# ylsung/vl-merging

Hardware: AMD Instinct MI355X
Metric: VL samples/sec (fwd+bwd) base_vl 384^2 at 1/2/4/8 GPUs; merge GB/s vs HBM peak (higher is better)
Workload: dtype bf16

## Files before the change

### include/vlm_hip.h

```cpp
#ifndef VLM_HIP_H
#define VLM_HIP_H
#include <stddef.h>
#include <stdint.h>

#ifdef __cplusplus
extern "C" {
#endif

#define VLM_OK 0
#define VLM_ERR_ARG (-1)
#define VLM_ERR_LAUNCH (-2)
#define VLM_ERR_WORKSPACE (-3)
#define VLM_ERR_UNSUPPORTED (-4)

#define VLM_ABI_VERSION 10
int vlm_abi_version(void);
int vlm_device_cus(void);
int vlm_set_cu_budget(int cus);
int vlm_debug_occupy(int workgroups, int threads, int lds_bytes, int microseconds, void* stream);

#define VLM_MERGE_LERP 0
#define VLM_MERGE_TASKVEC 1
#define VLM_MERGE_MEAN 2
#define VLM_MERGE_MAX_SRC 4
// ... 10 lines not shown

size_t vlm_merge_plan_bytes(int n_jobs, uint64_t total_elems);
int vlm_merge_plan_upload(const vlm_merge_job_t* jobs_host, int n_jobs, void* workspace, size_t workspace_bytes,
                          void* stream);
int vlm_merge_run(const void* workspace, void* stream);

#define VLM_ACT_NONE 0
#define VLM_ACT_GELU 1
#define VLM_ACT_GELU_BWD 2
#define VLM_ACT_GELU_DERIV 3
#define VLM_ACT_MUL_AUX 4

typedef struct {
  const float* bias;
  const float* col_scale;
  const float* row_scale;
  const float* residual;
  int64_t ld_res;
  void* aux;
  int64_t ld_aux;
  int32_t act;
  float alpha;
  int32_t accumulate;
  int32_t reserved;
  float* col_sum;
  float* col_sum_ws;
  float* splitk_ws;
  uint64_t splitk_ws_bytes;
} vlm_epilogue_t;

int vlm_gemm_bf16(int ta, int tb, int M, int N, int K, const void* A, int lda, const void* B, int ldb, void* C,
                  int ldc, int c_is_f32, const vlm_epilogue_t* epi, void* stream);
#define VLM_GEMM_MAX_GROUPS 4
typedef struct {
  int32_t row0, rows;
  const void* B;
  int32_t ldb;
  int32_t reserved;
  const float* bias;
  float* col_sum;
  float* col_sum_ws;
} vlm_gemm_group_t;
int vlm_gemm_bf16_grouped(int n_groups, const vlm_gemm_group_t* groups, int N, int K, const void* A, int lda, void* C,
                          int ldc, int c_is_f32, const vlm_epilogue_t* epi, void* stream);
typedef struct {
  int32_t row0, rows;
  float* C;
  int32_t accumulate;
  int32_t reserved;
} vlm_wgrad_group_t;
int vlm_gemm_wgrad_grouped(int n_groups, const vlm_wgrad_group_t* groups, int M, int N, const void* A, int lda,
                           const void* B, int ldb, int ldc, float* splitk_ws, uint64_t splitk_ws_bytes, void* stream);
int vlm_gemm_set_big_tile_mode(int mode);

int vlm_layernorm_fwd(const float* x, int ldx, int M, int D, const float* gamma, const float* beta, float eps,
                      void* y, int ldy, int y_is_f32, float* stats, void* stream);
#define VLM_ROW_WS_BYTES(D) ((size_t)1536 * 2 * (size_t)(D) * sizeof(float))
int vlm_layernorm_bwd(const void* dy, int lddy, int dy_is_f32, const float* x, int ldx, const float* stats,
                      const float* gamma, int M, int D, const float* dres, int lddres, float* dx, int lddx,
                      float* dgamma, float* dbeta, float* workspace, size_t workspace_bytes, int* deferred_blocks,
                      void* stream);
typedef struct {
  const void* y;
  int32_t ldy;
  const float* gamma;
  const float* row_scale;
  void* dy;
  int32_t lddy;
  float* dgamma;
  float* dbias;
  float* workspace;
  size_t workspace_bytes;
} vlm_layerscale_t;
int vlm_layernorm_bwd_scale(const void* dy, int lddy, int dy_is_f32, const float* x, int ldx, const float* stats,
                            const float* gamma, int M, int D, const float* dres, int lddres, float* dx, int lddx,
                            float* dgamma, float* dbeta, float* workspace, size_t workspace_bytes,
                            const vlm_layerscale_t* scale, int* deferred_blocks, void* stream);
#define VLM_MAX_FOLD_JOBS 16
typedef struct {
  const float* partials;
  int32_t nblocks;
  int32_t D;
  float* out0;
  float* out1;
} vlm_fold_job_t;
int vlm_colreduce_batch(const vlm_fold_job_t* jobs_host, int n_jobs, void* stream);
int vlm_layerscale_bwd(const float* dx, int lddx, const void* y_bf16, int ldy, const float* gamma,
                       const float* row_scale, int M, int D, void* dy_bf16, int lddy, float* dgamma, float* dbias,
                       float* workspace, size_t workspace_bytes, int* deferred_blocks, void* stream);
#define VLM_MAX_LAYERSCALE_JOBS 32
typedef struct {
  const float* weight;
  const float* gamma;
  const float* bias;
  void* shadow;
  float* bias_out;
  float* raw_w;
  float* raw_b;
  float* dweight;
  float* dbias;
  float* dgamma;
  int32_t N, K;
} vlm_layerscale_job_t;
int vlm_layerscale_fold(const vlm_layerscale_job_t* jobs_host, int n_jobs, void* stream);
int vlm_layerscale_finish(const vlm_layerscale_job_t* jobs_host, int n_jobs, void* stream);
int vlm_colsum_bf16(const void* a, int lda, int M, int N, float* out, void* stream);
// ... 125 lines not shown
```

### vl-merging_amd/_lib.py

```python
import ctypes
import os

_HERE = os.path.dirname(os.path.abspath(__file__))
LIB_PATH = os.environ.get("VLM_LIB_PATH") or os.path.join(_HERE, "lib", "libvlm_hip.so")
_lib = None

c_void_p = ctypes.c_void_p
c_int = ctypes.c_int
c_float = ctypes.c_float
c_size_t = ctypes.c_size_t
c_u64 = ctypes.c_uint64

MERGE_LERP, MERGE_TASKVEC, MERGE_MEAN = 0, 1, 2
MERGE_MAX_SRC = 4


class MergeJob(ctypes.Structure):
    _fields_ = [
        ("dst", c_void_p),
        ("base", c_void_p),
        ("src", c_void_p * MERGE_MAX_SRC),
        ("ratio", c_float * MERGE_MAX_SRC),
        ("n_src", ctypes.c_int32),
        ("mode", ctypes.c_int32),
# ... 57 lines not shown
        ("B", ctypes.c_int32), ("n0", ctypes.c_int32), ("n1", ctypes.c_int32), ("base0", ctypes.c_int32),
        ("base1", ctypes.c_int32), ("pos1", ctypes.c_int32), ("scale", c_float), ("reserved", ctypes.c_int32),
        ("bias_dense", c_void_p), ("bias_dense_t", c_void_p), ("dense_tiles", ctypes.c_int32), ("reserved2", ctypes.c_int32),
    ]


class LayerScaleJob(ctypes.Structure):
    _fields_ = [("weight", c_void_p), ("gamma", c_void_p), ("bias", c_void_p), ("shadow", c_void_p), ("bias_out", c_void_p),
                ("raw_w", c_void_p), ("raw_b", c_void_p), ("dweight", c_void_p), ("dbias", c_void_p), ("dgamma", c_void_p),
                ("N", ctypes.c_int32), ("K", ctypes.c_int32)]


MAX_LAYERSCALE_JOBS = 32


class VlmError(RuntimeError):
    pass


_ERR = {-1: "VLM_ERR_ARG", -2: "VLM_ERR_LAUNCH", -3: "VLM_ERR_WORKSPACE", -4: "VLM_ERR_UNSUPPORTED"}

SIGNATURES = {
    "vlm_abi_version": (c_int, []),
    "vlm_device_cus": (c_int, []),
    "vlm_set_cu_budget": (c_int, [c_int]),
    "vlm_debug_occupy": (c_int, [c_int, c_int, c_int, c_int, c_void_p]),
    "vlm_layerscale_fold": (c_int, [ctypes.POINTER(LayerScaleJob), c_int, c_void_p]),
    "vlm_layerscale_finish": (c_int, [ctypes.POINTER(LayerScaleJob), c_int, c_void_p]),
    "vlm_merge_plan_bytes": (c_size_t, [c_int, c_u64]),
    "vlm_merge_plan_upload": (c_int, [ctypes.POINTER(MergeJob), c_int, c_void_p, c_size_t, c_void_p]),
    "vlm_merge_run": (c_int, [c_void_p, c_void_p]),
    "vlm_gemm_bf16": (c_int, [c_int, c_int, c_int, c_int, c_int, c_void_p, c_int, c_void_p, c_int, c_void_p, c_int,
                              c_int, ctypes.POINTER(Epilogue), c_void_p]),
    "vlm_gemm_bf16_grouped": (c_int, [c_int, ctypes.POINTER(GemmGroup), c_int, c_int, c_void_p, c_int, c_void_p, c_int, c_int,
                                      ctypes.POINTER(Epilogue), c_void_p]),
    "vlm_gemm_wgrad_grouped": (c_int, [c_int, ctypes.POINTER(WgradGroup), c_int, c_int, c_void_p, c_int, c_void_p, c_int, c_int,
                                       c_void_p, c_u64, c_void_p]),
    "vlm_attention_fwd": (c_int, [ctypes.POINTER(AttnDesc), c_void_p, c_int, c_void_p, c_void_p]),
    "vlm_attention_bwd_ws_floats": (c_size_t, [ctypes.POINTER(AttnDesc), c_int]),
    "vlm_attention_bwd": (c_int, [ctypes.POINTER(AttnDesc), c_void_p, c_int, c_void_p, c_int, c_void_p, c_void_p, c_size_t,
                                  c_void_p, c_int, c_void_p, c_void_p, c_void_p]),
    "vlm_layernorm_fwd": (c_int, [c_void_p, c_int, c_int, c_int, c_void_p, c_void_p, c_float, c_void_p, c_int, c_int,
                                  c_void_p, c_void_p]),
    "vlm_layernorm_bwd": (c_int, [c_void_p, c_int, c_int, c_void_p, c_int, c_void_p, c_void_p, c_int, c_int, c_void_p,
                                  c_int, c_void_p, c_int, c_void_p, c_void_p, c_void_p, c_size_t,
                                  ctypes.POINTER(c_int), c_void_p]),
    "vlm_layernorm_bwd_scale": (c_int, [c_void_p, c_int, c_int, c_void_p, c_int, c_void_p, c_void_p, c_int, c_int, c_void_p,
                                        c_int, c_void_p, c_int, c_void_p, c_void_p, c_void_p, c_size_t,
                                        ctypes.POINTER(LayerScale), ctypes.POINTER(c_int), c_void_p]),
    "vlm_layerscale_bwd": (c_int, [c_void_p, c_int, c_void_p, c_int, c_void_p, c_void_p, c_int, c_int, c_void_p, c_int,
                                   c_void_p, c_void_p, c_void_p, c_size_t, ctypes.POINTER(c_int), c_void_p]),
    "vlm_colreduce_batch": (c_int, [ctypes.POINTER(FoldJob), c_int, c_void_p]),
    "vlm_gemm_set_big_tile_mode": (c_int, [c_int]),
    "vlm_colsum_bf16": (c_int, [c_void_p, c_int, c_int, c_int, c_void_p, c_void_p]),
    "vlm_adamw_step": (c_int, [c_void_p, c_void_p, c_void_p, c_void_p, c_void_p, c_u64, c_float, c_float, c_float,
                               c_float, c_float, c_float, c_float, c_int, c_void_p]),
    "vlm_accumulate_f32_f64": (c_int, [c_void_p, c_void_p, c_u64, c_void_p]),
    "vlm_gram_f64": (c_int, [c_void_p, c_int, c_int, c_int, c_int, c_void_p, c_void_p]),
    "vlm_gemm_f64": (c_int, [c_int, c_int, c_int, c_int, c_int, ctypes.c_double, c_void_p, c_int, c_int, c_void_p, c_int,
                             ctypes.c_double, c_void_p, c_int, c_void_p]),
    "vlm_scale_gram_f64": (c_int, [c_void_p, c_void_p, c_int, ctypes.c_double, c_int, c_void_p]),
    "vlm_potrf_block_f64": (c_int, [c_void_p, c_int, c_int, c_int, c_void_p, c_void_p]),
    "vlm_trsm_block_f64": (c_int, [c_void_p, c_int, c_int, c_int, c_int, c_void_p, c_int, c_int, c_int, c_void_p]),
    "vlm_cholesky_f64": (c_int, [c_void_p, c_int, c_void_p, c_void_p]),
    "vlm_solve_spd_right_f64": (c_int, [c_void_p, c_int, c_void_p, c_int, c_int, c_void_p]),
    "vlm_gemm_f64_batched": (c_int, [c_int, c_int, c_int, c_int, c_int, ctypes.c_double, ctypes.POINTER(c_void_p), c_int, c_int,
                                     ctypes.POINTER(c_void_p), c_int, ctypes.c_double, ctypes.POINTER(c_void_p), c_int, c_int, c_void_p]),
    "vlm_cholesky_f64_batched": (c_int, [ctypes.POINTER(c_void_p), c_int, c_int, c_void_p, c_void_p]),
    "vlm_solve_spd_right_f64_batched": (c_int, [ctypes.POINTER(c_void_p), c_int, ctypes.POINTER(c_void_p), c_int, c_int, c_int, c_void_p]),
    "vlm_cross_entropy_fwd": (c_int, [c_void_p, c_int, c_int, c_int, c_void_p, ctypes.c_int64, c_void_p, c_void_p, c_void_p]),
    "vlm_cross_entropy_bwd": (c_int, [c_void_p, c_int, c_int, c_int, c_void_p, ctypes.c_int64, c_void_p, c_void_p, c_void_p, c_int,
                                      c_void_p]),
    "vlm_l2norm_fwd": (c_int, [c_void_p, c_int, c_int, c_int, c_int, c_void_p, c_void_p, c_void_p]),
    "vlm_l2norm_bwd": (c_int, [c_void_p, c_void_p, c_void_p, c_int, c_int, c_void_p, c_int, c_int, c_void_p]),
    "vlm_contrastive_ws_floats": (c_size_t, [c_int]),
    "vlm_contrastive": (c_int, [c_void_p, c_void_p, c_int, c_int, c_int, c_void_p, c_void_p, c_void_p, c_void_p, c_void_p, c_void_p,
                                c_void_p]),
    "vlm_small_cross_entropy": (c_int, [c_void_p, c_int, c_int, c_int, c_int, c_void_p, c_void_p, c_void_p, c_void_p]),
    "vlm_cross_entropy_reduce": (c_int, [c_void_p, c_void_p, c_int, c_int, ctypes.c_int64, c_void_p, c_void_p]),
    "vlm_scale_by_scalar": (c_int, [ctypes.POINTER(c_void_p), ctypes.POINTER(c_void_p), ctypes.POINTER(c_int), c_int, c_void_p, c_void_p]),
    "vlm_text_rows_fwd": (c_int, [c_void_p, c_int, c_void_p, c_int, c_void_p, c_void_p, c_void_p, c_float, c_void_p, c_float, c_float,
                                  c_void_p, c_void_p, c_int, c_void_p, c_int, c_void_p]),
    "vlm_text_rows_bwd_ws_floats": (c_size_t, [c_int]),
    "vlm_text_rows_bwd": (c_int, [c_void_p, c_int, c_void_p, c_int, c_void_p, c_int, c_void_p, c_void_p, c_void_p, c_void_p, c_float, c_float,
                                  c_int, c_void_p, ctypes.c_int64, c_void_p, c_void_p, c_void_p, c_void_p, c_void_p, c_void_p]),
    "vlm_image_rows_prep": (c_int, [c_void_p, c_void_p, c_void_p, c_int, c_void_p, c_void_p]),
    "vlm_image_lead_rows": (c_int, [c_void_p, c_int, c_int, c_int, c_int, c_void_p, c_void_p]),
    "vlm_image_rows_bwd_ws_floats": (c_size_t, [c_int]),
    "vlm_image_rows_bwd": (c_int, [c_void_p, c_int, c_int, c_int, c_int, c_void_p, c_void_p, c_void_p, c_void_p, c_void_p, c_void_p]),
    "vlm_tanh_fwd": (c_int, [c_void_p, c_int, c_int, c_int, c_void_p, c_void_p]),
    "vlm_act_bwd": (c_int, [c_void_p, c_int, c_int, c_void_p, c_int, c_int, c_int, c_int, c_int, c_void_p, c_void_p]),
    "vlm_colsum_small": (c_int, [c_void_p, c_int, c_int, c_int, c_void_p, c_void_p]),
    "vlm_sample_negatives": (c_int, [c_void_p, c_int, c_int, c_void_p, c_int, c_int, c_int, c_int, c_void_p, c_void_p, c_void_p]),
    "vlm_weighted_sum": (c_int, [ctypes.POINTER(c_void_p), ctypes.POINTER(c_float), c_int, c_void_p, c_void_p]),
    "vlm_scatter_rows": (c_int, [c_void_p, c_int, c_int, c_int, c_int, c_void_p, c_int, c_void_p]),
    "vlm_cast_f32_bf16": (c_int, [c_void_p, c_void_p, c_u64, c_void_p]),
    "vlm_embedding_bwd": (c_int, [c_void_p, c_int, c_void_p, ctypes.c_int64, c_int, ctypes.c_int64, c_void_p, c_int,
                                  ctypes.c_int64, c_void_p]),
    "vlm_bias_dense_bytes": (c_size_t, [c_int, c_int, c_int, c_int]),
    "vlm_bias_dense": (c_int, [c_void_p, c_int, c_int, c_void_p, c_int, c_int, c_int, c_int, c_int, c_int, c_void_p,
                               c_void_p]),
    "vlm_transpose_bf16_tiles": (c_int, [c_void_p, c_int, c_void_p]),
    "vlm_droppath_sites": (c_int, [c_void_p, c_void_p, c_void_p, c_int, c_int, c_int, c_int, c_int, c_int, c_int, c_void_p,
                                   c_void_p]),
    "vlm_droppath_rows": (c_int, [c_void_p, c_float, c_int, c_int, c_int, c_int, c_int, c_void_p, c_void_p]),
    "vlm_patch_im2col": (c_int, [c_void_p, c_void_p, c_int, c_int, c_int, c_int, c_int, c_void_p]),
# ... 39 lines not shown
```

### vl-merging_amd/csrc/gemm.hip

```cpp
#include "vlm_common.h"
#include "vlm_diag.h"
#include <atomic>

#define GEMM_BM 128
#define GEMM_BN 128
#define GEMM_BK 64
#define GEMM_THREADS 256
#define GEMM_TILE_BYTES (GEMM_BM * GEMM_BK * 2)

typedef __attribute__((address_space(3))) s16x4 lds_s16x4;

__device__ __forceinline__ float gelu_cdf(float x, float& ez2) {
  const float t = __builtin_amdgcn_rcpf(fmaf(0.3275911f * 0.70710678118654752440f, fabsf(x), 1.0f));
  ez2 = __builtin_amdgcn_exp2f((x * x) * (-0.5f * 1.4426950408889634f));
  float poly = fmaf(t, 0.5f * 1.061405429f, 0.5f * -1.453152027f);
  poly = fmaf(t, poly, 0.5f * 1.421413741f);
  poly = fmaf(t, poly, 0.5f * -0.284496736f);
  poly = fmaf(t, poly, 0.5f * 0.254829592f);
  const float e = fmaf(-(poly * t), ez2, 0.5f);
  return 0.5f + copysignf(e, x);
}
__device__ __forceinline__ float gelu_erf(float x) {
  float ez2;
  return x * gelu_cdf(x, ez2);
// ... 853 lines not shown
    if (WR) { BIG_LWRITE(RSA, RSB, BUFA_W, BUFB_W) }                                     \
    if (GL) { BIG_GLOAD(RSA, RSB, (K) + 4) }                                             \
    if (RD) { BIG_READ(FNA, FNB, BUFA_R, BUFB_R) }                                       \
    BIG_MFMA(FCA, FCB)                                                                   \
    _Pragma("unroll") for (int g = 0; g < 16; ++g) {                                     \
      __builtin_amdgcn_sched_group_barrier(0x008, 2, 0);                                 \
      __builtin_amdgcn_sched_group_barrier(0x100, 1, 0);                                 \
    }                                                                                    \
    _Pragma("unroll") for (int g = 0; g < 8; ++g) {                                      \
      __builtin_amdgcn_sched_group_barrier(0x008, 2, 0);                                 \
      __builtin_amdgcn_sched_group_barrier(0x200, 1, 0);                                 \
      __builtin_amdgcn_sched_group_barrier(0x008, 2, 0);                                 \
      __builtin_amdgcn_sched_group_barrier(0x020, 1, 0);                                 \
    }                                                                                    \
    __builtin_amdgcn_sched_barrier(0);                                                   \
  }

  BIG_GLOAD(ra0, rb0, 0)
  BIG_GLOAD(ra1, rb1, 1)
  BIG_LWRITE(ra0, rb0, sA0, sB0)
  BIG_GLOAD(ra0, rb0, 2)
  BIG_LWRITE(ra1, rb1, sA1, sB1)
  BIG_GLOAD(ra1, rb1, 3)
  asm volatile("s_waitcnt lgkmcnt(0)" ::: "memory");
  __builtin_amdgcn_s_barrier();
  BIG_READ(fa0, fb0, sA0, sB0)
  GEMM_STAMP(1)

  int kt = 0;
  for (; kt < nk - 4; kt += 2) {
    BIG_STEP(kt + 0, 1, 1, 1, fa0, fb0, fa1, fb1, ra0, rb0, sA0, sB0, sA1, sB1)
    BIG_STEP(kt + 1, 1, 1, 1, fa1, fb1, fa0, fb0, ra1, rb1, sA1, sB1, sA0, sB0)
  }
#define BIG_TAIL_STEPS()                                                               \
  BIG_STEP(kt + 0, 0, 1, 1, fa0, fb0, fa1, fb1, ra0, rb0, sA0, sB0, sA1, sB1)          \
  BIG_STEP(kt + 1, 0, 1, 1, fa1, fb1, fa0, fb0, ra1, rb1, sA1, sB1, sA0, sB0)          \
  BIG_STEP(kt + 2, 0, 0, 1, fa0, fb0, fa1, fb1, ra0, rb0, sA0, sB0, sA1, sB1)          \
  BIG_STEP(kt + 3, 0, 0, 0, fa1, fb1, fa0, fb0, ra1, rb1, sA1, sB1, sA0, sB0)
  if constexpr (DEEP) {
    BIG_TAIL_STEPS()
    GEMM_STAMP(2)
    big_epilogue_t<OUT_F32, RES, AUX> ep(p, wl, mw0, nw0, lane);
    float* ws_row = (p.epi.col_sum_ws && mw0 + 128 <= (uint32_t)p.M) ? p.epi.col_sum_ws + ((size_t)(tm_ws * 2 + wm) * 2) * p.N : nullptr;
    BIG_EPILOGUE_LOOP_DEEP(AHEAD)
    ep.finish(lane, ws_row);
  } else {
    EPIL_SETUP()
    BIG_TAIL_STEPS()
    GEMM_STAMP(2)
    float* ws_row = (p.epi.col_sum_ws && mw0 + 128 <= (uint32_t)p.M) ? p.epi.col_sum_ws + ((size_t)(tm_ws * 2 + wm) * 2) * p.N : nullptr;
    BIG_EPILOGUE_LOOP()
    ep.finish(lane, ws_row);
  }
  GEMM_STAMP_END()
}

template <bool GROUPED = false>
__global__ __launch_bounds__(GEMM_THREADS, 1) void vlm_gemm_bigT_kernel(const gemm_params_t p) {
  __shared__ __attribute__((aligned(1024))) unsigned char sA0[BIG_OP_BYTES], sA1[BIG_OP_BYTES], sB0[BIG_OP_BYTES], sB1[BIG_OP_BYTES];
  __shared__ __attribute__((aligned(16))) unsigned char epl[4 * EPIL_WAVE_BYTES];
  const int tid = threadIdx.x;
  const int lane = tid & 63;
  const int wave = __builtin_amdgcn_readfirstlane(tid >> 6);
  const int wm = wave >> 1, wn = wave & 1;
  const uint32_t ntile = p.tiles_m * p.tiles_n;
  const uint32_t q8 = gridDim.x >> 3, r8 = gridDim.x & 7, xcd = blockIdx.x & 7;
  uint32_t item = (xcd < r8 ? xcd * (q8 + 1) : r8 * (q8 + 1) + (xcd - r8) * q8) + (blockIdx.x >> 3);
  uint32_t k_base = 0, k_end = (uint32_t)p.K, slice0 = 0;
  int nk = p.ksteps_per_split;
  if constexpr (GROUPED) {
    int g = 0;
#pragma unroll
    for (int i = 1; i < VLM_GEMM_MAX_GROUPS; ++i)
      if (i < p.n_groups && item >= (uint32_t)p.grpT[i].item0) g = i;
    const gemmT_group_t G = p.grpT[g];
    item -= (uint32_t)G.item0;
    k_base = (uint32_t)G.row0;
    k_end = (uint32_t)G.row_end;
    nk = G.kps;
    slice0 = (uint32_t)G.slice0;
  }
  const uint32_t split = item / ntile, tile = item - split * ntile;
  const uint32_t tm = tile / p.tiles_n, tn = tile - tm * p.tiles_n;
  const uint32_t m0 = tm * BIG_BM, n0 = tn * BIG_BN;
  const uint32_t k_first = k_base + split * (uint32_t)nk * BIG_BK;
  const __amdgpu_buffer_rsrc_t ra =
      __builtin_amdgcn_make_buffer_rsrc(const_cast<void*>(p.A), 0, (int)((uint64_t)k_end * p.lda * 2), 0x00020000);
  const __amdgpu_buffer_rsrc_t rb =
      __builtin_amdgcn_make_buffer_rsrc(const_cast<void*>(p.B), 0, (int)((uint64_t)k_end * p.ldb * 2), 0x00020000);

  uint32_t offa[4], offb[4], wr_off[4];
#pragma unroll
  for (int u = 0; u < 4; ++u) {
    const uint32_t row = 2 * (wave + 4 * u) + (lane >> 5), c16 = lane & 31;
    offa[u] = ((k_first + row) * (uint32_t)p.lda + m0 + c16 * 8) * 2;
    offb[u] = ((k_first + row) * (uint32_t)p.ldb + n0 + c16 * 8) * 2;
    wr_off[u] = row * 512 + (((c16 >> 1) ^ ((row & 3) | (((row >> 3) & 1) << 2))) << 5) + (c16 & 1) * 16;
  }
  uint32_t rda[8], rdb[8];
  {
    const uint32_t g = lane >> 4, q = (lane & 15) >> 2, pp = lane & 3, sw = q | ((g & 1) << 2);
#pragma unroll
    for (int i = 0; i < 8; ++i) {
      rda[i] = (8 * g + q) * 512 + wm * 256 + ((i ^ sw) << 5) + 8 * pp;
      rdb[i] = (8 * g + q) * 512 + wn * 256 + ((i ^ sw) << 5) + 8 * pp;
    }
// ... 114 lines not shown

static bool epi_vec8(const vlm_epilogue_t* e, int ldc, int c_is_f32) {
  const bool v4 = ((ldc & 3) == 0) && (!e->aux || (e->ld_aux & 3) == 0) && (!e->residual || (e->ld_res & 3) == 0);
  return v4 && (c_is_f32 || (ldc & 7) == 0) && (!e->aux || ((e->ld_aux & 7) == 0 && ((uintptr_t)e->aux & 15) == 0)) &&
         (!e->residual || ((uintptr_t)e->residual & 15) == 0) && (!e->bias || ((uintptr_t)e->bias & 15) == 0) &&
         (!e->col_scale || ((uintptr_t)e->col_scale & 15) == 0);
}

static bool epi_off32(const vlm_epilogue_t* e, int M, int lda, int ldc) {
  return (uint64_t)M * ldc * 4 < (1ull << 31) && (!e->residual || (uint64_t)M * e->ld_res * 4 < (1ull << 31)) &&
         (!e->aux || (uint64_t)M * e->ld_aux * 2 < (1ull << 31)) && (uint64_t)M * lda * 2 < (1ull << 31);
}

static int launch_gemm_bigT(gemm_params_t p, const vlm_epilogue_t* epi, hipStream_t stream) {
  if (!epi->splitk_ws || (p.N % BIG_BN) || (p.ldc % 4)) return 1;
  if ((uint64_t)p.M * p.N * 4 >= (1ull << 31)) return 1;
  p.tiles_m = (p.M + BIG_BM - 1) / BIG_BM;
  p.tiles_n = (p.N + BIG_BN - 1) / BIG_BN;
  const int ntile = p.tiles_m * p.tiles_n, nk = (p.K + BIG_BK - 1) / BIG_BK;
  int splits = plan_cus() / ntile;
  if (splits < 1) splits = 1;
  if (splits > nk / 16) splits = nk / 16;
  if (splits < 1) return 1;
  int kps = (nk + splits - 1) / splits;
  kps += kps & 1;
  if (kps < 4) kps = 4;
  splits = (nk + kps - 1) / kps;
  if ((size_t)splits * p.M * p.N * 4 > (size_t)epi->splitk_ws_bytes) return 1;
  p.ksteps_per_split = kps;
  p.splits = splits;
  float* const out = reinterpret_cast<float*>(p.C);
  const int ldc = p.ldc;
  p.C = epi->splitk_ws;
  hipLaunchKernelGGL(vlm_gemm_bigT_kernel<false>, dim3(ntile * splits), dim3(GEMM_THREADS), 0, stream, p);
  VLM_CHECK_LAUNCH();
  const size_t per = (size_t)p.M * p.N / 4;
  hipLaunchKernelGGL(splitk_reduce_kernel, dim3((unsigned)((per + 255) / 256)), dim3(256), 0, stream,
                     reinterpret_cast<const float*>(epi->splitk_ws), splits, p.M, p.N, out, ldc, epi->accumulate);
  VLM_CHECK_LAUNCH();
  return VLM_OK;
}

template <bool OUT_F32, bool RES, int AUX, bool GROUPED = false>
static int launch_gemm_big(gemm_params_t p, hipStream_t stream) {
  if (!GROUPED) p.tiles_m = (p.M + BIG_BM - 1) / BIG_BM;
  p.tiles_n = (p.N + BIG_BN - 1) / BIG_BN;
  p.group_m = p.tiles_n >= 6 ? 4 : 1;
  GEMM_STAMP_ARM(p)
  hipLaunchKernelGGL((vlm_gemm_big_kernel<OUT_F32, RES, AUX, GROUPED>), dim3(p.tiles_m * p.tiles_n), dim3(GEMM_THREADS), 0, stream, p);
  VLM_CHECK_LAUNCH();
  return VLM_OK;
}

template <bool GROUPED = false>
static int launch_gemm_big_variant(const gemm_params_t& p, bool c_is_f32, hipStream_t s) {
  const vlm_epilogue_t& e = p.epi;
  const bool res = e.residual != nullptr;
  const int aux = e.aux ? ((e.act == VLM_ACT_GELU_BWD || e.act == VLM_ACT_MUL_AUX) ? 2 : 1) : 0;
  if (e.row_scale && !res) return 1;
  {
    bool any_cs = e.col_sum != nullptr;
    if (GROUPED)
      for (int g = 0; g < p.n_groups; ++g) any_cs = any_cs || p.grp[g].col_sum != nullptr;
    if (e.alpha != 1.0f || (e.col_scale && !res) || (any_cs && aux != 2)) return 1;
  }
  if (!c_is_f32 && !res) {
    if (aux == 0) return launch_gemm_big<false, false, 0, GROUPED>(p, s);
    if (aux == 1) return launch_gemm_big<false, false, 1, GROUPED>(p, s);
    return launch_gemm_big<false, false, 2, GROUPED>(p, s);
  }
  if (c_is_f32 && aux != 2) {
    if (res && aux) return launch_gemm_big<true, true, 1, GROUPED>(p, s);
    if (res) return launch_gemm_big<true, true, 0, GROUPED>(p, s);
    if (GROUPED) return 1;
    if (aux == 0) return launch_gemm_big<true, false, 0>(p, s);
  }
  return 1;
}

static std::atomic<int> g_big_mode{1};
static int gemm_big_mode() { return g_big_mode.load(std::memory_order_relaxed); }
extern "C" int vlm_gemm_set_big_tile_mode(int mode) {
  if (mode < -1 || mode > 2) return VLM_ERR_ARG;
  g_big_mode.store(mode < 0 ? 1 : mode, std::memory_order_relaxed);
  return VLM_OK;
}


extern "C" int vlm_gemm_bf16(int ta, int tb, int M, int N, int K, const void* A, int lda, const void* B, int ldb,
                             void* C, int ldc, int c_is_f32, const vlm_epilogue_t* epi, void* stream) {
  if (M < 0 || N < 0 || K < 0 || !C) return VLM_ERR_ARG;
  if (M == 0 || N == 0) return VLM_OK;
  if (!A || !B || !epi) return VLM_ERR_ARG;
  if ((lda & 7) || (ldb & 7) || ((uintptr_t)A & 15) || ((uintptr_t)B & 15)) return VLM_ERR_ARG;
  if ((!ta || !tb) && (K % GEMM_BK)) return VLM_ERR_UNSUPPORTED;
  if (((ldc & 3) == 0) && ((uintptr_t)C & 15)) return VLM_ERR_ARG;
  if (epi->accumulate && !c_is_f32) return VLM_ERR_ARG;
  if ((epi->act == VLM_ACT_GELU_BWD || epi->act == VLM_ACT_MUL_AUX || epi->act == VLM_ACT_GELU_DERIV) && !epi->aux) return VLM_ERR_ARG;
  if (epi->act < VLM_ACT_NONE || epi->act > VLM_ACT_MUL_AUX) return VLM_ERR_ARG;
  if (epi->col_sum_ws && (!epi->col_sum || (N % GEMM_BN) != 0 || ta)) return VLM_ERR_ARG;
  const uint64_t a_bytes = (uint64_t)(ta ? K : M) * lda * 2, b_bytes = (uint64_t)(tb ? K : N) * ldb * 2;
  if (a_bytes >= (1ull << 31) || b_bytes >= (1ull << 31)) return VLM_ERR_UNSUPPORTED;
  gemm_params_t p;
  p.A = A; p.B = B; p.C = C;
  p.M = M; p.N = N; p.K = K;
  p.lda = lda; p.ldb = ldb; p.ldc = ldc;
  p.epi = *epi;
  p.epi.reserved = epi_vec8(epi, ldc, c_is_f32) ? 1 : 0;
  if (epi->col_sum_ws && !p.epi.reserved) return VLM_ERR_ARG;
  p.tiles_m = (M + GEMM_BM - 1) / GEMM_BM;
  p.tiles_n = (N + GEMM_BN - 1) / GEMM_BN;
  p.splits = 1;
  p.ksteps_per_split = 0;
  p.n_groups = 0;
  p.group_m = p.tiles_n >= 12 ? 8 : 1;
  GEMM_STAMP_ARM(p)
  hipStream_t s = (hipStream_t)stream;
  const int ntile = p.tiles_m * p.tiles_n, nk = (K + GEMM_BK - 1) / GEMM_BK;
  const bool plain_acc = epi->accumulate && c_is_f32 && !epi->bias && !epi->col_scale && !epi->row_scale &&
                         !epi->residual && !epi->aux && !epi->col_sum && epi->act == VLM_ACT_NONE;
  if (gemm_big_mode() > 0 && ta && tb && c_is_f32 && !epi->bias && !epi->col_scale && !epi->row_scale && !epi->residual &&
      !epi->aux && !epi->col_sum && epi->act == VLM_ACT_NONE && K >= 2048) {
    const int rc = launch_gemm_bigT(p, epi, s);
    if (rc <= 0) return rc;
  }
  if (tb && plain_acc && ntile < 512 && nk >= 32) {
    int splits = 2 * plan_cus() / ntile;
    if (splits < 1) splits = 1;
    if (splits > nk / 8) splits = nk / 8;
    if (splits > 1) {
      p.ksteps_per_split = (nk + splits - 1) / splits;
      p.splits = (nk + p.ksteps_per_split - 1) / p.ksteps_per_split;
      p.group_m = p.tiles_n >= 12 ? 1 : 4;
      if (ta) return launch_gemm<true, true, true, true>(p, s);
      return launch_gemm<false, true, true, true>(p, s);
    }
  }
  if (!ta && !tb && (K % (4 * BIG_BK)) == 0 && gemm_big_mode() > 0) {
    const long big_tiles = (long)((M + BIG_BM - 1) / BIG_BM) * ((N + BIG_BN - 1) / BIG_BN);
    const bool ws_ok = (N % BIG_BN) == 0 && p.epi.reserved == 1 && epi_off32(epi, M, lda, ldc) && !epi->accumulate;
    if (ws_ok && (gemm_big_mode() >= 2 || 2 * big_tiles >= plan_cus())) {
      const int rc = launch_gemm_big_variant<>(p, c_is_f32 != 0, s);
      if (rc <= 0) return rc;
    }
  }
#ifdef GEMM_ONLY_BIG
  return VLM_ERR_UNSUPPORTED;
#endif
  const int key = (ta ? 4 : 0) | (tb ? 2 : 0) | (c_is_f32 ? 1 : 0);
  switch (key) {
    case 0: return launch_gemm<false, false, false, false>(p, s);
    case 1: return launch_gemm<false, false, true, false>(p, s);
    case 2: return launch_gemm<false, true, false, false>(p, s);
    case 3: return launch_gemm<false, true, true, false>(p, s);
    case 4: return launch_gemm<true, false, false, false>(p, s);
    case 5: return launch_gemm<true, false, true, false>(p, s);
    case 6: return launch_gemm<true, true, false, false>(p, s);
    default: return launch_gemm<true, true, true, false>(p, s);
  }
}

extern "C" int vlm_gemm_bf16_grouped(int n_groups, const vlm_gemm_group_t* groups, int N, int K, const void* A, int lda, void* C,
                                     int ldc, int c_is_f32, const vlm_epilogue_t* epi, void* stream) {
  if (n_groups < 1 || n_groups > VLM_GEMM_MAX_GROUPS || !groups || N < 0 || K < 0 || !C || !epi) return VLM_ERR_ARG;
  if (epi->bias || epi->col_sum || epi->col_sum_ws || epi->splitk_ws) return VLM_ERR_ARG;
  int prev_end = 0;
  for (int g = 0; g < n_groups; ++g) {
    const vlm_gemm_group_t& G = groups[g];
    if (G.row0 < prev_end || G.rows < 0 || !G.B || (G.col_sum_ws && !G.col_sum)) return VLM_ERR_ARG;
    prev_end = G.row0 + G.rows;
  }
  const int M_total = prev_end;
  if (M_total == 0 || N == 0) return VLM_OK;
  if (!A) return VLM_ERR_ARG;
  hipStream_t s = (hipStream_t)stream;
  bool big = gemm_big_mode() > 0 && (K % (4 * BIG_BK)) == 0 && (N % BIG_BN) == 0 && !epi->accumulate && (lda & 7) == 0 &&
             ((uintptr_t)A & 15) == 0 && ((uintptr_t)C & 15) == 0 && epi_vec8(epi, ldc, c_is_f32) && epi_off32(epi, M_total, lda, ldc);
  gemm_params_t p;
  p.A = A; p.B = nullptr; p.C = C;
  p.M = M_total; p.N = N; p.K = K;
  p.lda = lda; p.ldb = 0; p.ldc = ldc;
  p.epi = *epi;
  p.epi.reserved = 1;
  p.splits = 1;
  p.ksteps_per_split = 0;
  p.n_groups = 0;
  int tiles = 0;
  for (int g = 0; g < n_groups && big; ++g) {
    const vlm_gemm_group_t& G = groups[g];
    if (G.rows == 0) continue;
    if ((G.ldb & 7) || ((uintptr_t)G.B & 15) || (uint64_t)N * G.ldb * 2 >= (1ull << 31) || (G.bias && ((uintptr_t)G.bias & 15))) big = false;
    gemm_group_t& D = p.grp[p.n_groups++];
    D.B = G.B; D.bias = G.bias; D.col_sum = G.col_sum; D.col_sum_ws = G.col_sum_ws;
    D.ldb = G.ldb; D.row0 = G.row0; D.row_end = G.row0 + G.rows; D.tile0 = tiles;
    tiles += (G.rows + BIG_BM - 1) / BIG_BM;
  }
  if (big && p.n_groups >= 1) {
    p.tiles_m = tiles;
    if (gemm_big_mode() >= 2 || 2l * tiles * (N / BIG_BN) >= plan_cus()) {
      const int rc = launch_gemm_big_variant<true>(p, c_is_f32 != 0, s);
      if (rc <= 0) return rc;
    }
  }
  for (int g = 0; g < n_groups; ++g) {
    const vlm_gemm_group_t& G = groups[g];
    if (G.rows == 0) continue;
    vlm_epilogue_t e = *epi;
    const size_t r0 = (size_t)G.row0;
    e.bias = G.bias; e.col_sum = G.col_sum; e.col_sum_ws = G.col_sum_ws;
    if (e.residual) e.residual += r0 * e.ld_res;
    if (e.aux) e.aux = reinterpret_cast<unsigned char*>(e.aux) + r0 * e.ld_aux * 2;
    if (e.row_scale) e.row_scale += r0;
    const int rc = vlm_gemm_bf16(0, 0, G.rows, N, K, reinterpret_cast<const unsigned char*>(A) + r0 * lda * 2, lda, G.B, G.ldb,
                                 reinterpret_cast<unsigned char*>(C) + r0 * ldc * (c_is_f32 ? 4 : 2), ldc, c_is_f32, &e, stream);
    if (rc) return rc;
  }
  return VLM_OK;
}

extern "C" int vlm_gemm_wgrad_grouped(int n_groups, const vlm_wgrad_group_t* groups, int M, int N, const void* A, int lda,
                                      const void* B, int ldb, int ldc, float* splitk_ws, uint64_t splitk_ws_bytes, void* stream) {
  if (n_groups < 1 || n_groups > VLM_GEMM_MAX_GROUPS || !groups || M < 0 || N < 0) return VLM_ERR_ARG;
  int prev_end = 0;
  for (int g = 0; g < n_groups; ++g) {
    if (groups[g].row0 < prev_end || groups[g].rows < 0 || !groups[g].C) return VLM_ERR_ARG;
    prev_end = groups[g].row0 + groups[g].rows;
  }
  if (M == 0 || N == 0) return VLM_OK;
  if (!A || !B || (lda & 7) || (ldb & 7) || ((uintptr_t)A & 15) || ((uintptr_t)B & 15)) return VLM_ERR_ARG;
  hipStream_t s = (hipStream_t)stream;
  for (int g = 0; g < n_groups; ++g)
    if (groups[g].rows == 0 && !groups[g].accumulate &&
        hipMemset2DAsync(groups[g].C, (size_t)ldc * 4, 0, (size_t)N * 4, M, s) != hipSuccess)
      return VLM_ERR_LAUNCH;
  const int K_total = prev_end;
  bool big = gemm_big_mode() > 0 && splitk_ws && (N % BIG_BN) == 0 && (ldc % 4) == 0 && (uint64_t)M * N * 4 < (1ull << 31) &&
             (uint64_t)K_total * lda * 2 < (1ull << 31) && (uint64_t)K_total * ldb * 2 < (1ull << 31);
  gemm_params_t p;
  p.A = A; p.B = B; p.C = splitk_ws;
  p.M = M; p.N = N; p.K = K_total;
  p.lda = lda; p.ldb = ldb; p.ldc = N;
  p.epi = vlm_epilogue_t{};
  p.epi.alpha = 1.0f;
  p.epi.reserved = 1;
  p.tiles_m = (M + BIG_BM - 1) / BIG_BM;
  p.tiles_n = (N + BIG_BN - 1) / BIG_BN;
  p.group_m = 1;
  p.splits = 1;
  p.ksteps_per_split = 0;
  p.n_groups = 0;
  splitk_groups_t rg{};
  if (big) {
    const int ntile = p.tiles_m * p.tiles_n;
// ... 60 lines not shown
```

Baseline: 342.1.

## Add 224-row big GEMM tile variant with wave-quantization-aware planner

Adds a new GEMM kernel whose tiles are 224 rows tall instead of 256, along with a planner. The planner estimates per-CU wave counts for both tile heights and picks 224 when the tail-wave cost drops enough, using a fixed relative tile-time constant. The goal is to cut wave quantization waste for row counts such as a 384^2 token batch. It adds register-heavy code paths and new template instantiations, and it relies on a hand-tuned cost model that can choose badly.

Result: no change. 342.2, median of 4 (+0.0%).

```diff
diff --git a/include/vlm_hip.h b/include/vlm_hip.h
--- a/include/vlm_hip.h
+++ b/include/vlm_hip.h
@@ -86,6 +86,9 @@
 int vlm_gemm_wgrad_grouped(int n_groups, const vlm_wgrad_group_t* groups, int M, int N, const void* A, int lda,
                            const void* B, int ldb, int ldc, float* splitk_ws, uint64_t splitk_ws_bytes, void* stream);
 int vlm_gemm_set_big_tile_mode(int mode);
+int vlm_gemm_set_big_rows(int rows);
+int vlm_gemm_plan_big_rows(int n_groups, const vlm_gemm_group_t* groups, int N, int c_is_f32, const vlm_epilogue_t* epi,
+                           int cus, int32_t* tiles_m);
 
 int vlm_layernorm_fwd(const float* x, int ldx, int M, int D, const float* gamma, const float* beta, float eps,
                       void* y, int ldy, int y_is_f32, float* stats, void* stream);
diff --git a/vl-merging_amd/_lib.py b/vl-merging_amd/_lib.py
--- a/vl-merging_amd/_lib.py
+++ b/vl-merging_amd/_lib.py
@@ -133,6 +133,9 @@
                                    c_void_p, c_void_p, c_void_p, c_size_t, ctypes.POINTER(c_int), c_void_p]),
     "vlm_colreduce_batch": (c_int, [ctypes.POINTER(FoldJob), c_int, c_void_p]),
     "vlm_gemm_set_big_tile_mode": (c_int, [c_int]),
+    "vlm_gemm_set_big_rows": (c_int, [c_int]),
+    "vlm_gemm_plan_big_rows": (c_int, [c_int, ctypes.POINTER(GemmGroup), c_int, c_int, ctypes.POINTER(Epilogue), c_int,
+                                       ctypes.POINTER(c_int)]),
     "vlm_colsum_bf16": (c_int, [c_void_p, c_int, c_int, c_int, c_void_p, c_void_p]),
     "vlm_adamw_step": (c_int, [c_void_p, c_void_p, c_void_p, c_void_p, c_void_p, c_u64, c_float, c_float, c_float,
                                c_float, c_float, c_float, c_float, c_int, c_void_p]),
diff --git a/vl-merging_amd/csrc/gemm.hip b/vl-merging_amd/csrc/gemm.hip
--- a/vl-merging_amd/csrc/gemm.hip
+++ b/vl-merging_amd/csrc/gemm.hip
@@ -929,6 +929,179 @@
     BIG_EPILOGUE_LOOP()
     ep.finish(lane, ws_row);
   }
+  GEMM_STAMP_END()
+}
+
+template <int ROWS, bool OUT_F32, bool RES, int AUX, bool GROUPED = false>
+__global__ __launch_bounds__(GEMM_THREADS, 1) void vlm_gemm_rows_kernel(const gemm_params_t p_in) {
+  static_assert(ROWS == 224, "one row height besides 256");
+  static_assert(AUX != 2, "the GELU'-argument variant keeps 256 rows");
+  constexpr int WR = ROWS / 2, NF = WR / 16, NF1 = NF - 4;
+  constexpr int NSTAGE = ROWS / 16;
+  __shared__ __attribute__((aligned(1024))) unsigned char sA0[BIG_OP_BYTES], sA1[BIG_OP_BYTES], sB0[BIG_OP_BYTES], sB1[BIG_OP_BYTES];
+  __shared__ __attribute__((aligned(16))) unsigned char epl[4 * EPIL_WAVE_BYTES];
+  const int tid = threadIdx.x;
+  const int lane = tid & 63;
+  const int wave = __builtin_amdgcn_readfirstlane(tid >> 6);
+  const int wm = wave >> 1, wn = wave & 1;
+
+  const uint32_t nblk = gridDim.x, bid = blockIdx.x;
+  const uint32_t q8 = nblk >> 3, r8 = nblk & 7, xcd = bid & 7;
+  const uint32_t tile = (xcd < r8 ? xcd * (q8 + 1) : r8 * (q8 + 1) + (xcd - r8) * q8) + (bid >> 3);
+  uint32_t tm, tn;
+  {
+    const uint32_t gm = (uint32_t)p_in.group_m, gsz = gm * p_in.tiles_n, grp = tile / gsz, first = grp * gm;
+    const uint32_t rows = min(gm, (uint32_t)p_in.tiles_m - first), in = tile - grp * gsz;
+    tm = first + in % rows;
+    tn = in / rows;
+  }
+  gemm_params_t p_grp;
+  uint32_t m0 = tm * ROWS;
+  if constexpr (GROUPED) {
+    p_grp = p_in;
+    int g = 0;
+#pragma unroll
+    for (int i = 1; i < VLM_GEMM_MAX_GROUPS; ++i)
+      if (i < p_in.n_groups && tm >= (uint32_t)p_in.grp[i].tile0) g = i;
+    const gemm_group_t G = p_in.grp[g];
+    m0 = (uint32_t)G.row0 + (tm - (uint32_t)G.tile0) * ROWS;
+    p_grp.M = G.row_end;
+    p_grp.B = G.B;
+    p_grp.ldb = G.ldb;
+    p_grp.epi.bias = G.bias;
+  }
+  const gemm_params_t& p = GROUPED ? p_grp : p_in;
+  GEMM_STAMP(0)
+  const uint32_t n0 = tn * BIG_BN;
+  const __amdgpu_buffer_rsrc_t ra =
+      __builtin_amdgcn_make_buffer_rsrc(const_cast<void*>(p.A), 0, (int)((uint64_t)p.M * p.lda * 2), 0x00020000);
+  const __amdgpu_buffer_rsrc_t rb =
+      __builtin_amdgcn_make_buffer_rsrc(const_cast<void*>(p.B), 0, (int)((uint64_t)p.N * p.ldb * 2), 0x00020000);
+
+  uint32_t offa[4], offb[4];
+  {
+    const uint32_t chunk = (lane & 3) ^ big_swz(lane >> 4);
+#pragma unroll
+    for (int u = 0; u < 4; ++u) {
+      const uint32_t row = (wave + 4 * u) * 16 + (lane >> 2);
+      offa[u] = ((m0 + row) * (uint32_t)p.lda + chunk * 8) * 2;
+      offb[u] = ((n0 + row) * (uint32_t)p.ldb + chunk * 8) * 2;
+    }
+  }
+  const uint32_t rd_slot = ((uint32_t)(lane >> 4) ^ big_swz((lane & 15) >> 2)) * 16 + (lane & 15) * 64;
+  const uint32_t rda = wm * WR * 64 + rd_slot, rdb = wn * 128 * 64 + rd_slot;
+
+  f32x4 acc00[4][4], acc01[4][4], acc10[NF1][4], acc11[NF1][4];
+#pragma unroll
+  for (int i = 0; i < 4; ++i)
+#pragma unroll
+    for (int j = 0; j < 4; ++j) {
+      acc00[i][j] = (f32x4){0.f, 0.f, 0.f, 0.f};
+      acc01[i][j] = (f32x4){0.f, 0.f, 0.f, 0.f};
+      if (i < NF1) {
+        acc10[i][j] = (f32x4){0.f, 0.f, 0.f, 0.f};
+        acc11[i][j] = (f32x4){0.f, 0.f, 0.f, 0.f};
+      }
+    }
+
+  const int nk = p.K / BIG_BK;
+  const uint32_t mw0 = m0 + wm * WR, nw0 = n0 + wn * 128;
+  unsigned char* const wl = epl + wave * EPIL_WAVE_BYTES;
+  bf16x8 fa0[NF], fb0[8], fa1[NF], fb1[8];
+
+#define ROWS_READ(FA, FB, SA, SB)                                                         \
+  _Pragma("unroll") for (int i = 0; i < 8; ++i) {                                         \
+    if (i < NF) FA[i] = *reinterpret_cast<const bf16x8*>((SA) + rda + i * 1024);           \
+    FB[i] = *reinterpret_cast<const bf16x8*>((SB) + rdb + i * 1024);                      \
+  }
+#define ROWS_MFMA_Q(ACC, FA, FB, I0, J0, NI)                                                                            \
+  _Pragma("unroll") for (int i = 0; i < (NI); ++i) _Pragma("unroll") for (int j = 0; j < 4; ++j)                       \
+      ACC[i][j] = __builtin_amdgcn_mfma_f32_16x16x32_bf16(FB[(J0) + j], FA[(I0) + i], ACC[i][j], 0, 0, 0);
+#define ROWS_MFMA(FA, FB)               \
+  ROWS_MFMA_Q(acc00, FA, FB, 0, 0, 4)   \
+  ROWS_MFMA_Q(acc01, FA, FB, 0, 4, 4)   \
+  ROWS_MFMA_Q(acc11, FA, FB, 4, 4, NF1) \
+  ROWS_MFMA_Q(acc10, FA, FB, 4, 0, NF1)
+  uint32_t wr_off[4];
+  {
+    const uint32_t slot = (lane & 3) ^ big_swz(lane >> 4);
+#pragma unroll
+    for (int u = 0; u < 4; ++u) wr_off[u] = ((wave + 4 * u) * 16 + (lane >> 2)) * 64 + slot * 16;
+  }
+  {
+    const uint32_t unswz = (((lane & 3) ^ big_swz(lane >> 4)) - (lane & 3)) * 16;
+#pragma unroll
+    for (int u = 0; u < 4; ++u) { offa[u] -= unswz; offb[u] -= unswz; }
+  }
+#pragma unroll
+  for (int u = 0; u < 4; ++u)
+    if (wave + 4 * u >= NSTAGE) offa[u] = 0x80000000u;
+  u32x4 ra0[4], rb0[4], ra1[4], rb1[4];
+#define ROWS_STEP(K, GL, WR_, RD, FCA, FCB, FNA, FNB, RSA, RSB, BUFA_W, BUFB_W, BUFA_R, BUFB_R) \
+  {                                                                                       \
+    if (RD) {                                                                             \
+      asm volatile("s_waitcnt lgkmcnt(0)" ::: "memory");                                  \
+      __builtin_amdgcn_s_barrier();                                                       \
+    }                                                                                     \
+    __builtin_amdgcn_sched_barrier(0);                                                    \
+    if (WR_) { BIG_LWRITE(RSA, RSB, BUFA_W, BUFB_W) }                                     \
+    if (GL) { BIG_GLOAD(RSA, RSB, (K) + 4) }                                              \
+    if (RD) { ROWS_READ(FNA, FNB, BUFA_R, BUFB_R) }                                       \
+    ROWS_MFMA(FCA, FCB)                                                                   \
+    _Pragma("unroll") for (int g = 0; g < NF + 8; ++g) {                                  \
+      __builtin_amdgcn_sched_group_barrier(0x008, 2, 0);                                  \
+      __builtin_amdgcn_sched_group_barrier(0x100, 1, 0);                                  \
+    }                                                                                     \
+    _Pragma("unroll") for (int g = 0; g < 8; ++g) {                                       \
+      __builtin_amdgcn_sched_group_barrier(0x008, 2, 0);                                  \
+      __builtin_amdgcn_sched_group_barrier(0x200, 1, 0);                                  \
+      __builtin_amdgcn_sched_group_barrier(0x008, 1, 0);                                  \
+      __builtin_amdgcn_sched_group_barrier(0x020, 1, 0);                                  \
+    }                                                                                     \
+    __builtin_amdgcn_sched_barrier(0);                                                    \
+  }
+
+  BIG_GLOAD(ra0, rb0, 0)
+  BIG_GLOAD(ra1, rb1, 1)
+  BIG_LWRITE(ra0, rb0, sA0, sB0)
+  BIG_GLOAD(ra0, rb0, 2)
+  BIG_LWRITE(ra1, rb1, sA1, sB1)
+  BIG_GLOAD(ra1, rb1, 3)
+  asm volatile("s_waitcnt lgkmcnt(0)" ::: "memory");
+  __builtin_amdgcn_s_barrier();
+  ROWS_READ(fa0, fb0, sA0, sB0)
+  GEMM_STAMP(1)
+
+  int kt = 0;
+  for (; kt < nk - 4; kt += 2) {
+    ROWS_STEP(kt + 0, 1, 1, 1, fa0, fb0, fa1, fb1, ra0, rb0, sA0, sB0, sA1, sB1)
+    ROWS_STEP(kt + 1, 1, 1, 1, fa1, fb1, fa0, fb0, ra1, rb1, sA1, sB1, sA0, sB0)
+  }
+  big_epilogue_t<OUT_F32, RES, AUX> ep(p, wl, mw0, nw0, lane);
+  epil_in_t inA, inB;
+  ep.load_inputs(inA, 0);
+  ROWS_STEP(kt + 0, 0, 1, 1, fa0, fb0, fa1, fb1, ra0, rb0, sA0, sB0, sA1, sB1)
+  ROWS_STEP(kt + 1, 0, 1, 1, fa1, fb1, fa0, fb0, ra1, rb1, sA1, sB1, sA0, sB0)
+  ROWS_STEP(kt + 2, 0, 0, 1, fa0, fb0, fa1, fb1, ra0, rb0, sA0, sB0, sA1, sB1)
+  ROWS_STEP(kt + 3, 0, 0, 0, fa1, fb1, fa0, fb0, ra1, rb1, sA1, sB1, sA0, sB0)
+  GEMM_STAMP(2)
+  static_assert(NF == 7, "trip layout below");
+  unsigned char* wr = wl + (lane & 15) * EPIL_PITCH + (lane >> 4) * 16;
+  ep.load_inputs(inB, 1);
+#pragma unroll 1
+  for (int q = 0; q < NF / 2; ++q) {
+    switch (q) {
+      case 0: EPIL_DUMP_ROW(acc00, acc01, 0, 0) EPIL_DUMP_ROW(acc00, acc01, 1, 16 * EPIL_PITCH) break;
+      case 1: EPIL_DUMP_ROW(acc00, acc01, 2, 0) EPIL_DUMP_ROW(acc00, acc01, 3, 16 * EPIL_PITCH) break;
+      default: EPIL_DUMP_ROW(acc10, acc11, 0, 0) EPIL_DUMP_ROW(acc10, acc11, 1, 16 * EPIL_PITCH) break;
+    }
+    ep.process(inA, 2 * q, 0);
+    ep.load_inputs(inA, 2 * q + 2);
+    ep.process(inB, 2 * q + 1, 16 * EPIL_PITCH);
+    ep.load_inputs(inB, q < NF / 2 - 1 ? 2 * q + 3 : NF - 1);
+  }
+  EPIL_DUMP_ROW(acc10, acc11, NF1 - 1, 0)
+  ep.process(inA, NF - 1, 0);
   GEMM_STAMP_END()
 }
 
@@ -1149,8 +1322,26 @@
   return VLM_OK;
 }
 
+template <int ROWS, bool OUT_F32, bool RES, int AUX, bool GROUPED = false>
+static int launch_gemm_rows(gemm_params_t p, hipStream_t stream) {
+  if (!GROUPED) p.tiles_m = (p.M + ROWS - 1) / ROWS;
+  p.tiles_n = (p.N + BIG_BN - 1) / BIG_BN;
+  p.group_m = p.tiles_n >= 6 ? 4 : 1;
+  GEMM_STAMP_ARM(p)
+  hipLaunchKernelGGL((vlm_gemm_rows_kernel<ROWS, OUT_F32, RES, AUX, GROUPED>), dim3(p.tiles_m * p.tiles_n), dim3(GEMM_THREADS), 0,
+                     stream, p);
+  VLM_CHECK_LAUNCH();
+  return VLM_OK;
+}
+
+static bool rows_variant(const vlm_epilogue_t* e, int c_is_f32, bool any_col_sum) {
+  const bool res = e->residual != nullptr;
+  const bool aux2 = e->aux && (e->act == VLM_ACT_GELU_BWD || e->act == VLM_ACT_MUL_AUX);
+  return !any_col_sum && !e->col_sum_ws && !aux2 && (c_is_f32 != 0) == res;
+}
+
 template <bool GROUPED = false>
-static int launch_gemm_big_variant(const gemm_params_t& p, bool c_is_f32, hipStream_t s) {
+static int launch_gemm_big_variant(const gemm_params_t& p, bool c_is_f32, int rows, hipStream_t s) {
   const vlm_epilogue_t& e = p.epi;
   const bool res = e.residual != nullptr;
   const int aux = e.aux ? ((e.act == VLM_ACT_GELU_BWD || e.act == VLM_ACT_MUL_AUX) ? 2 : 1) : 0;
@@ -1161,14 +1352,15 @@
       for (int g = 0; g < p.n_groups; ++g) any_cs = any_cs || p.grp[g].col_sum != nullptr;
     if (e.alpha != 1.0f || (e.col_scale && !res) || (any_cs && aux != 2)) return 1;
   }
+  const bool r224 = rows == 224;
   if (!c_is_f32 && !res) {
-    if (aux == 0) return launch_gemm_big<false, false, 0, GROUPED>(p, s);
-    if (aux == 1) return launch_gemm_big<false, false, 1, GROUPED>(p, s);
+    if (aux == 0) return r224 ? launch_gemm_rows<224, false, false, 0, GROUPED>(p, s) : launch_gemm_big<false, false, 0, GROUPED>(p, s);
+    if (aux == 1) return r224 ? launch_gemm_rows<224, false, false, 1, GROUPED>(p, s) : launch_gemm_big<false, false, 1, GROUPED>(p, s);
     return launch_gemm_big<false, false, 2, GROUPED>(p, s);
   }
   if (c_is_f32 && aux != 2) {
-    if (res && aux) return launch_gemm_big<true, true, 1, GROUPED>(p, s);
-    if (res) return launch_gemm_big<true, true, 0, GROUPED>(p, s);
+    if (res && aux) return r224 ? launch_gemm_rows<224, true, true, 1, GROUPED>(p, s) : launch_gemm_big<true, true, 1, GROUPED>(p, s);
+    if (res) return r224 ? launch_gemm_rows<224, true, true, 0, GROUPED>(p, s) : launch_gemm_big<true, true, 0, GROUPED>(p, s);
     if (GROUPED) return 1;
     if (aux == 0) return launch_gemm_big<true, false, 0>(p, s);
   }
@@ -1181,6 +1373,47 @@
   if (mode < -1 || mode > 2) return VLM_ERR_ARG;
   g_big_mode.store(mode < 0 ? 1 : mode, std::memory_order_relaxed);
   return VLM_OK;
+}
+
+static std::atomic<int> g_big_rows{-1};
+extern "C" int vlm_gemm_set_big_rows(int rows) {
+  if (rows != -1 && rows != 256 && rows != 224) return VLM_ERR_ARG;
+  g_big_rows.store(rows, std::memory_order_relaxed);
+  return VLM_OK;
+}
+
+#define ROWS224_TILE_TIME 950
+#define ROWS_MARGIN 30
+
+static int big_rows_plan(int n_groups, const int* rows, int N, bool variant_ok, int cus, int* tiles_m) {
+  long t256 = 0, t224 = 0;
+  for (int g = 0; g < n_groups; ++g) {
+    t256 += (rows[g] + 255) / 256;
+    t224 += (rows[g] + 223) / 224;
+  }
+  const long tn = (N + BIG_BN - 1) / BIG_BN;
+  int h = 256;
+  const int forced = g_big_rows.load(std::memory_order_relaxed);
+  if (variant_ok && forced > 0) {
+    h = forced;
+  } else if (variant_ok && cus > 0) {
+    const long c256 = (t256 * tn + cus - 1) / cus * 1000, c224 = (t224 * tn + cus - 1) / cus * ROWS224_TILE_TIME;
+    if (c224 * 1000 <= c256 * (1000 - ROWS_MARGIN)) h = 224;
+  }
+  if (tiles_m) *tiles_m = (int)(h == 224 ? t224 : t256);
+  return h;
+}
+
+extern "C" int vlm_gemm_plan_big_rows(int n_groups, const vlm_gemm_group_t* groups, int N, int c_is_f32, const vlm_epilogue_t* epi,
+                                      int cus, int* tiles_m) {
+  if (n_groups < 1 || n_groups > VLM_GEMM_MAX_GROUPS || !groups || !epi || N < 0) return VLM_ERR_ARG;
+  int rows[VLM_GEMM_MAX_GROUPS];
+  bool any_cs = epi->col_sum != nullptr;
+  for (int g = 0; g < n_groups; ++g) {
+    rows[g] = groups[g].rows;
+    any_cs = any_cs || groups[g].col_sum != nullptr;
+  }
+  return big_rows_plan(n_groups, rows, N, rows_variant(epi, c_is_f32, any_cs), cus > 0 ? cus : plan_cus(), tiles_m);
 }
 
 
@@ -1237,7 +1470,8 @@
     const long big_tiles = (long)((M + BIG_BM - 1) / BIG_BM) * ((N + BIG_BN - 1) / BIG_BN);
     const bool ws_ok = (N % BIG_BN) == 0 && p.epi.reserved == 1 && epi_off32(epi, M, lda, ldc) && !epi->accumulate;
     if (ws_ok && (gemm_big_mode() >= 2 || 2 * big_tiles >= plan_cus())) {
-      const int rc = launch_gemm_big_variant<>(p, c_is_f32 != 0, s);
+      const int rows = big_rows_plan(1, &M, N, rows_variant(epi, c_is_f32, epi->col_sum != nullptr), plan_cus(), nullptr);
+      const int rc = launch_gemm_big_variant<>(p, c_is_f32 != 0, rows, s);
       if (rc <= 0) return rc;
     }
   }
@@ -1282,7 +1516,18 @@
   p.splits = 1;
   p.ksteps_per_split = 0;
   p.n_groups = 0;
-  int tiles = 0;
+  int rows = 256, tiles = 0, tiles256 = 0;
+  {
+    int grows[VLM_GEMM_MAX_GROUPS], ng = 0;
+    bool any_cs = false;
+    for (int g = 0; g < n_groups; ++g) {
+      if (groups[g].rows == 0) continue;
+      grows[ng++] = groups[g].rows;
+      any_cs = any_cs || groups[g].col_sum != nullptr;
+      tiles256 += (groups[g].rows + BIG_BM - 1) / BIG_BM;
+    }
+    if (big && ng > 0) rows = big_rows_plan(ng, grows, N, rows_variant(epi, c_is_f32, any_cs), plan_cus(), nullptr);
+  }
   for (int g = 0; g < n_groups && big; ++g) {
     const vlm_gemm_group_t& G = groups[g];
     if (G.rows == 0) continue;
@@ -1290,12 +1535,12 @@
     gemm_group_t& D = p.grp[p.n_groups++];
     D.B = G.B; D.bias = G.bias; D.col_sum = G.col_sum; D.col_sum_ws = G.col_sum_ws;
     D.ldb = G.ldb; D.row0 = G.row0; D.row_end = G.row0 + G.rows; D.tile0 = tiles;
-    tiles += (G.rows + BIG_BM - 1) / BIG_BM;
+    tiles += (G.rows + rows - 1) / rows;
   }
   if (big && p.n_groups >= 1) {
     p.tiles_m = tiles;
-    if (gemm_big_mode() >= 2 || 2l * tiles * (N / BIG_BN) >= plan_cus()) {
-      const int rc = launch_gemm_big_variant<true>(p, c_is_f32 != 0, s);
+    if (gemm_big_mode() >= 2 || 2l * tiles256 * (N / BIG_BN) >= plan_cus()) {
+      const int rc = launch_gemm_big_variant<true>(p, c_is_f32 != 0, rows, s);
       if (rc <= 0) return rc;
     }
   }
```
